# Bhumbra/probayes

Measured on AMD Instinct MI355X. Metric: MH chain-steps/sec (whole node), 10-dim model, 65 536 chains, 1/2/4/8 GPU, higher is better.
Workload: dtype f64; 1 GPU; cfg2: 10-dim diagonal-Gaussian random-walk MH, 65536 chains/GPU, full trace every step; chains_per_gpu=65536, dim=10, trace=True, steps_per_launch=250, parallelism=chain-sharded x1

## Files before the change

### include/pbhip.h

```cpp
#ifndef PBHIP_H
#define PBHIP_H

#include <stdint.h>

#ifdef __cplusplus
extern "C" {
#endif

#define PBH_ABI_VERSION 7
#define PBH_ABI_REVISION 2
#define PBH_MAX_DIM 32

#define PBH_OK 0
#define PBH_ERR_ARG (-1)
#define PBH_ERR_HIP (-2)
#define PBH_ERR_STATE (-3)
#define PBH_ERR_UNSUPPORTED (-4)
#define PBH_ERR_RCCL (-5)

enum pbh_target_kind {
  PBH_TARGET_DIAG_GAUSS = 1,
  PBH_TARGET_NORM_IID = 2,
  PBH_TARGET_GMM = 3,
  PBH_TARGET_NORM_PDF = 4,
// ... 138 lines not shown
int pbh_upload_replay(pbh_engine *eng, int64_t n_steps, const double *rand);
int pbh_stream_width(pbh_engine *eng, int32_t *r);
int pbh_legacy_seed(pbh_engine *eng, const uint32_t *seeds);
int pbh_legacy_replay(pbh_engine *eng, int64_t n_steps);
int pbh_reserve_replay(pbh_engine *eng, int64_t n_steps);
int pbh_get_replay(pbh_engine *eng, int64_t first, int64_t n_steps,
                   int32_t draw, double *out);
int pbh_legacy_run(pbh_engine *eng, int64_t n_steps, int32_t steps_per_launch);
int pbh_set_record_threshold(pbh_engine *eng, int32_t on);
int pbh_get_thresholds(pbh_engine *eng, int64_t first, int64_t n_steps, double *out);
enum pbh_draws { PBH_DRAWS_GAUSS = 0, PBH_DRAWS_LINREG = 1 };
int pbh_legacy_draws(pbh_engine *eng, int64_t n_steps, int64_t step0, int32_t kind,
                     double param, double *out);

enum { PBH_TRACE_NOFILL = 0x100 };
int pbh_alloc_trace(pbh_engine *eng, int64_t capacity, int32_t thin,
                    int32_t debug);
int pbh_run(pbh_engine *eng, int64_t n_steps, int32_t steps_per_launch);
int pbh_sync(pbh_engine *eng);
int pbh_run_wait(pbh_engine *eng, int64_t n_steps, int32_t steps_per_launch);
int pbh_set_collect(pbh_engine *eng, int32_t flags);
int pbh_last_run_ms(pbh_engine *eng, double *ms, int64_t *launches);
int pbh_server_stop(pbh_engine *eng);
int pbh_server_info(pbh_engine *eng, int32_t *active, int64_t *commands,
                    int64_t *launches);
int pbh_server_stamps(pbh_engine *eng, int32_t cap, uint32_t *seq, uint64_t *t0,
                      uint64_t *t1, int32_t *n);

int pbh_get_state(pbh_engine *eng, double *x, double *logp);
int pbh_trace_len(pbh_engine *eng, int64_t *n_recorded);
int pbh_get_trace(pbh_engine *eng, int64_t first, int64_t n, double *x,
                  double *logp, uint64_t *acc, double *p_x, double *p_p,
                  double *s);
int pbh_get_moments(pbh_engine *eng, double *sum, double *sumsq,
                    int64_t *n_acc, int64_t *n_steps);
int pbh_reset_moments(pbh_engine *eng);
int pbh_trace_ess(pbh_engine *eng, int64_t first, int64_t count, double *ess);
int pbh_trace_ess_total(pbh_engine *eng, int64_t first, int64_t count, double *total);
int pbh_trace_stats(pbh_engine *eng, int64_t first, int64_t count, double *sum,
                    double *sumsq, int64_t *n_acc);
int pbh_trace_expectation(pbh_engine *eng, int64_t first, int64_t count,
                          double exponent, double *out);
#define PBH_QUANTILE_MAX_RECORDS 2048
#define PBH_QUANTILE_MAX_Q 64
int pbh_trace_quantile(pbh_engine *eng, int64_t first, int64_t count,
                       int32_t nq, const double *q, int32_t weighted,
                       double *out);
int pbh_trace_rhat(pbh_engine *eng, int64_t first, int64_t count, int32_t group,
                   double *split_rhat, double *nested_rhat, double *chain_stats);
int pbh_trace_quantile_pooled(pbh_engine *eng, int64_t first, int64_t count,
                              int32_t nq, const double *q, double *out,
                              double *order_stats);

int pbh_trace_rhat_rank(pbh_engine *eng, int64_t first, int64_t count,
                        double *bulk, double *folded, double *ranks,
                        double *folded_ranks);

#define PBH_ESS_RANK_MAX_HALF 2048
int pbh_trace_ess_rank(pbh_engine *eng, int64_t first, int64_t count,
                       double *bulk, double *tail, double *tail_parts,
                       double *basic, double *mean_acov);

int pbh_rccl_unique_id(uint8_t id[128]);
int pbh_rccl_init(pbh_engine *eng, int32_t rank, int32_t world,
                  const uint8_t id[128]);
int pbh_rccl_max_chains(pbh_engine *eng, int64_t *n_max);
// ... 41 lines not shown
```

### probayes_amd/_lib.py

```python
import ctypes
import os

_HERE = os.path.dirname(os.path.abspath(__file__))
LIB_PATH = os.environ.get('PBHIP_LIB', os.path.join(_HERE, 'libpbhip.so'))

ABI_VERSION = 7
ABI_REVISION = 2
DRAWS_GAUSS, DRAWS_LINREG = 0, 1
MAX_DIM = 32

TARGET = {'diag_gauss': 1, 'norm_iid': 2, 'gmm': 3, 'norm_pdf': 4,
          'uniform_pdf': 5, 'mvn': 6, 'expr': 7}
PSCALE = {'log': 0, 'lin': 1}
SCORES = {'hastings': 1, 'metropolis': 2, 'gibbs': 3}
TRAN = {'const': 1, 'gauss_pdf': 2}
PROPOSAL = {'gauss': 1, 'sphere': 2, 'uniform': 3, 'gibbs': 4, 'vardelta': 5}
VAR_FIXED, VAR_POLARITY, VAR_UNIFORM, VAR_RANDINT = 0, 1, 2, 3
RNG = {'replay': 0, 'philox': 1, 'philox_f64': 2, 'xoshiro': 3,
       'philox_fp32': 4}
COLLECT_MOMENTS = 1

_dp = ctypes.POINTER(ctypes.c_double)
_ip = ctypes.POINTER(ctypes.c_int32)
_u8p = ctypes.POINTER(ctypes.c_uint8)
# ... 61 lines not shown
    'pbh_upload_replay': (ctypes.c_int, [ctypes.c_void_p, ctypes.c_int64, _dp]),
    'pbh_stream_width': (ctypes.c_int, [ctypes.c_void_p, _ip]),
    'pbh_legacy_seed': (ctypes.c_int, [ctypes.c_void_p, _u32p]),
    'pbh_legacy_replay': (ctypes.c_int, [ctypes.c_void_p, ctypes.c_int64]),
    'pbh_reserve_replay': (ctypes.c_int, [ctypes.c_void_p, ctypes.c_int64]),
    'pbh_legacy_run': (ctypes.c_int, [ctypes.c_void_p, ctypes.c_int64, ctypes.c_int32]),
    'pbh_set_record_threshold': (ctypes.c_int, [ctypes.c_void_p, ctypes.c_int32]),
    'pbh_get_thresholds': (ctypes.c_int, [ctypes.c_void_p, ctypes.c_int64,
                                          ctypes.c_int64, _dp]),
    'pbh_legacy_draws': (ctypes.c_int, [ctypes.c_void_p, ctypes.c_int64, ctypes.c_int64,
                                        ctypes.c_int32, ctypes.c_double, _dp]),
    'pbh_get_replay': (ctypes.c_int, [ctypes.c_void_p, ctypes.c_int64,
                                      ctypes.c_int64, ctypes.c_int32, _dp]),
    'pbh_alloc_trace': (ctypes.c_int, [ctypes.c_void_p, ctypes.c_int64,
                                       ctypes.c_int32, ctypes.c_int32]),
    'pbh_run': (ctypes.c_int, [ctypes.c_void_p, ctypes.c_int64, ctypes.c_int32]),
    'pbh_sync': (ctypes.c_int, [ctypes.c_void_p]),
    'pbh_run_wait': (ctypes.c_int, [ctypes.c_void_p, ctypes.c_int64, ctypes.c_int32]),
    'pbh_trace_ess_total': (ctypes.c_int, [ctypes.c_void_p, ctypes.c_int64,
                                           ctypes.c_int64, _dp]),
    'pbh_set_collect': (ctypes.c_int, [ctypes.c_void_p, ctypes.c_int32]),
    'pbh_last_run_ms': (ctypes.c_int, [ctypes.c_void_p, _dp, _i64p]),
    'pbh_server_stop': (ctypes.c_int, [ctypes.c_void_p]),
    'pbh_get_chain_logs': (ctypes.c_int, [ctypes.c_void_p, _dp, _ip]),
    'pbh_set_chain_logs': (ctypes.c_int, [ctypes.c_void_p, _dp]),
    'pbh_server_info': (ctypes.c_int, [ctypes.c_void_p, _ip, _i64p, _i64p]),
    'pbh_server_stamps': (ctypes.c_int, [ctypes.c_void_p, ctypes.c_int32, _u32p,
                                         _u64p, _u64p, _ip]),
    'pbh_get_state': (ctypes.c_int, [ctypes.c_void_p, _dp, _dp]),
    'pbh_trace_len': (ctypes.c_int, [ctypes.c_void_p, _i64p]),
    'pbh_get_trace': (ctypes.c_int, [ctypes.c_void_p, ctypes.c_int64,
                                     ctypes.c_int64, _dp, _dp, _u64p, _dp, _dp,
                                     _dp]),
    'pbh_get_moments': (ctypes.c_int, [ctypes.c_void_p, _dp, _dp, _i64p, _i64p]),
    'pbh_reset_moments': (ctypes.c_int, [ctypes.c_void_p]),
    'pbh_trace_stats': (ctypes.c_int, [ctypes.c_void_p, ctypes.c_int64,
                                       ctypes.c_int64, _dp, _dp, _i64p]),
    'pbh_rccl_unique_id': (ctypes.c_int, [_u8p]),
    'pbh_rccl_init': (ctypes.c_int, [ctypes.c_void_p, ctypes.c_int32,
                                     ctypes.c_int32, _u8p]),
    'pbh_rccl_max_chains': (ctypes.c_int, [ctypes.c_void_p, _i64p]),
    'pbh_rccl_allgather_stats': (ctypes.c_int, [ctypes.c_void_p, _dp, _i64p]),
    'pbh_get_checkpoint': (ctypes.c_int, [ctypes.c_void_p, _dp, _dp,
                                          ctypes.POINTER(ctypes.c_int64),
                                          ctypes.POINTER(ctypes.c_int32),
                                          _u32p]),
    'pbh_restore': (ctypes.c_int, [ctypes.c_void_p, _dp, _dp, ctypes.c_int64,
                                   ctypes.c_int32, _u32p]),
    'pbh_set_chains': (ctypes.c_int, [ctypes.c_void_p, _dp, _dp, ctypes.c_int64,
                                      ctypes.c_int32]),
    'pbh_legacy_state_words': (ctypes.c_int, [ctypes.c_void_p,
                                              ctypes.POINTER(ctypes.c_int64)]),
    'pbh_get_legacy_state': (ctypes.c_int, [ctypes.c_void_p, _u32p, _i32p, _i32p,
                                            _dp]),
    'pbh_set_legacy_state': (ctypes.c_int, [ctypes.c_void_p, _u32p, _i32p, _i32p,
                                            _dp]),
    'pbh_trace_expectation': (ctypes.c_int, [ctypes.c_void_p, ctypes.c_int64,
                                             ctypes.c_int64, ctypes.c_double,
                                             _dp]),
    'pbh_trace_quantile': (ctypes.c_int, [ctypes.c_void_p, ctypes.c_int64,
                                          ctypes.c_int64, ctypes.c_int32, _dp,
                                          ctypes.c_int32, _dp]),
    'pbh_trace_rhat': (ctypes.c_int, [ctypes.c_void_p, ctypes.c_int64,
                                      ctypes.c_int64, ctypes.c_int32, _dp, _dp,
                                      _dp]),
    'pbh_trace_quantile_pooled': (ctypes.c_int, [ctypes.c_void_p, ctypes.c_int64,
# ... 82 lines not shown
```

### probayes_amd/csrc/pbh_device.h

```cpp
#pragma once
#include <hip/hip_runtime.h>
#include <stdint.h>

#include "pbh_philox.h"

namespace pbh {

constexpr double kNearlyPosZero = 2.2250738585072014e-308;
constexpr double kNearlyPosInf = 1.7976931348623158e+308;
constexpr double kNearlyNegInf = -1.7976931348623158e+308;


__device__ __forceinline__ u32x4 philox4x32_10(u32x4 c, uint32_t k0,
                                                uint32_t k1) {
  constexpr uint32_t M0 = 0xD2511F53u, M1 = 0xCD9E8D57u;
  constexpr uint32_t W0 = 0x9E3779B9u, W1 = 0xBB67AE85u;
#pragma unroll
  for (int i = 0; i < 10; ++i) {
    const uint64_t p0 = (uint64_t)M0 * c.x;
    const uint64_t p1 = (uint64_t)M1 * c.z;
    const uint32_t hi0 = (uint32_t)(p0 >> 32), lo0 = (uint32_t)p0;
    const uint32_t hi1 = (uint32_t)(p1 >> 32), lo1 = (uint32_t)p1;
    c = u32x4{(uint32_t)__builtin_amdgcn_bitop3_b32(hi1, c.y, k0, 0x96), lo1,
              (uint32_t)__builtin_amdgcn_bitop3_b32(hi0, c.w, k1, 0x96), lo0};
// ... 365 lines not shown
}

__device__ __forceinline__ void st_buf(double *base, uint32_t voff,
                                       uint32_t soff, double v) {
  typedef unsigned int u32x2_t __attribute__((__vector_size__(8)));
  const __amdgpu_buffer_rsrc_t rs =
      __builtin_amdgcn_make_buffer_rsrc(base, 0, -1, 0x00020000);
  __builtin_amdgcn_raw_buffer_store_b64(__builtin_bit_cast(u32x2_t, v), rs,
                                        (int)voff, (int)soff, 2);
}

constexpr uint32_t kNoStore = 0x80000000u;
__device__ __forceinline__ void st_buf_n(double *base, uint32_t nbytes,
                                         uint32_t voff, double v) {
  typedef unsigned int u32x2_t __attribute__((__vector_size__(8)));
  const __amdgpu_buffer_rsrc_t rs =
      __builtin_amdgcn_make_buffer_rsrc(base, 0, (int)nbytes, 0x00020000);
  __builtin_amdgcn_raw_buffer_store_b64(__builtin_bit_cast(u32x2_t, v), rs,
                                        (int)voff, 0, 2);
}
__device__ __forceinline__ void st_buf_ns(double *base, uint32_t nbytes, uint32_t voff,
                                          uint32_t soff, double v) {
  typedef unsigned int u32x2_t __attribute__((__vector_size__(8)));
  const __amdgpu_buffer_rsrc_t rs =
      __builtin_amdgcn_make_buffer_rsrc(base, 0, (int)nbytes, 0x00020000);
  __builtin_amdgcn_raw_buffer_store_b64(__builtin_bit_cast(u32x2_t, v), rs,
                                        (int)voff, (int)soff, 2);
}
__device__ __forceinline__ void st_buf32_n(uint32_t *base, uint32_t nbytes,
                                           uint32_t voff, uint32_t v) {
  const __amdgpu_buffer_rsrc_t rs =
      __builtin_amdgcn_make_buffer_rsrc(base, 0, (int)nbytes, 0x00020000);
  __builtin_amdgcn_raw_buffer_store_b32(v, rs, (int)voff, 0, 0);
}

__device__ __forceinline__ uint32_t sel_u32(uint64_t m, uint32_t if0, uint32_t if1) {
  uint32_t r;
  asm("v_cndmask_b32_e64 %0, %1, %2, %3" : "=v"(r) : "v"(if0), "v"(if1), "s"(m));
  return r;
}
__device__ __forceinline__ double sel_f64(uint64_t m, double if0, double if1) {
  const uint64_t a = __builtin_bit_cast(uint64_t, if0), b = __builtin_bit_cast(uint64_t, if1);
  const uint32_t lo = sel_u32(m, (uint32_t)a, (uint32_t)b);
  const uint32_t hi = sel_u32(m, (uint32_t)(a >> 32), (uint32_t)(b >> 32));
  return __builtin_bit_cast(double, ((uint64_t)hi << 32) | lo);
}
__device__ __forceinline__ float sel_f32(uint64_t m, float if0, float if1) {
  return __builtin_bit_cast(float, sel_u32(m, __builtin_bit_cast(uint32_t, if0),
                                           __builtin_bit_cast(uint32_t, if1)));
}

__device__ __forceinline__ double lo_closed(double lo, bool incl) {
  if (incl || lo != lo) return lo;
  if (lo == __builtin_inf()) return __builtin_nan("");
  if (lo == 0.) return 0x1p-1074;
  const int64_t b = __builtin_bit_cast(int64_t, lo);
  return __builtin_bit_cast(double, lo > 0. ? b + 1 : b - 1);
}
__device__ __forceinline__ double hi_closed(double hi, bool incl) {
  if (incl || hi != hi) return hi;
  if (hi == -__builtin_inf()) return __builtin_nan("");
  if (hi == 0.) return -0x1p-1074;
  const int64_t b = __builtin_bit_cast(int64_t, hi);
  return __builtin_bit_cast(double, hi > 0. ? b - 1 : b + 1);
}

// ... 313 lines not shown
```

### probayes_amd/csrc/pbh_kernels_impl.h

```cpp
#pragma once
#include <utility>

#include "pbh_kernels.h"
#include "pbh_device.h"
#include "../../include/pbhip.h"

namespace pbh {

namespace {

constexpr int kBlock = 256;
constexpr int kPairFullBlock = 512;

__device__ __forceinline__ double cld(const double *p, int64_t i) {
  return ((const __attribute__((address_space(4))) double *)p)[i];
}

__device__ __forceinline__ double uni(double v) {
  const uint64_t u = __builtin_bit_cast(uint64_t, v);
  const uint32_t lo = __builtin_amdgcn_readfirstlane((uint32_t)u);
  const uint32_t hi = __builtin_amdgcn_readfirstlane((uint32_t)(u >> 32));
  return __builtin_bit_cast(double, (uint64_t)lo | ((uint64_t)hi << 32));
}

// ... 1152 lines not shown
    double cA[H], cB[H];
    uint32_t ctA = 0, ctB = 0, t1 = 0;
    int s = 0;
    if constexpr (PD::F32) {
      double nA[H], nB[H];
      uint32_t ntA = 0, ntB = 0;
      PD::draw(a, s_bmt, h, a.g0 >> 1, chain, cA, cB, ctA, ctB);
      if ((a.g0 & 1) && s < a.n_steps) {
        step(s, cB, ctB, t1);
        ++s;
        if (s < a.n_steps)
          PD::draw(a, s_bmt, h, (a.g0 + s) >> 1, chain, cA, cB, ctA, ctB);
      }
      for (; s + 3 < a.n_steps; s += 4) {
        PD::draw(a, s_bmt, h, ((a.g0 + s) >> 1) + 1, chain, nA, nB, ntA, ntB);
        step(s, cA, ctA, t1);
        step(s + 1, cB, ctB, t1);
        PD::draw(a, s_bmt, h, ((a.g0 + s) >> 1) + 2, chain, cA, cB, ctA, ctB);
        step(s + 2, nA, ntA, t1);
        step(s + 3, nB, ntB, t1);
      }
      if (s + 1 < a.n_steps) {
        step(s, cA, ctA, t1);
        step(s + 1, cB, ctB, t1);
        s += 2;
        if (s < a.n_steps)
          PD::draw(a, s_bmt, h, (a.g0 + s) >> 1, chain, cA, cB, ctA, ctB);
      }
      if (s < a.n_steps) step(s, cA, ctA, t1);
    } else if constexpr (FULL) {
        int64_t g0v = a.g0;
        int32_t nsv = a.n_steps, fairv = a.fair, fair_relv = a.fair_rel;
        constexpr int NW = 3 * H + 1, NB = (NW + 3) / 4, QA = (H + 1) / 2;
        constexpr uint64_t kHi = 0xFFFFFFFF00000000ull;
        uint64_t inl = __ballot(__builtin_fabs(lp) <= 700.);
        const uint32_t lpoff = hi ? loff : kNoStore;
        const uint32_t lpbytes = (uint32_t)(a.n * 8);
        const uint32_t aoff = lane == 32 ? (uint32_t)((c >> 5) * 4) : kNoStore;
        const uint32_t abytes = (uint32_t)(a.W * 8);
        int64_t rec = g0v + s - a.rec_base;
        const PhiloxKeys rk = philox_keys_v(a.seed_lo, a.seed_hi);
        uint32_t pre_hi = (uint32_t)((uint64_t)g0v >> 33);
        PhiloxPrefix<NB> pre =
            philox_prefix<NB>(16u * (uint32_t)h, chain, pre_hi, a.seed_lo, a.seed_hi);
        auto philox_from = [&](int64_t P, uint32_t (&w)[4 * NB], auto Q0) {
          philox_prefix_blocks<NB, decltype(Q0)::value>((uint32_t)P, pre, rk, w);
        };
        auto philox = [&](int64_t P, uint32_t (&w)[4 * NB]) {
          philox_prefix_blocks<NB>((uint32_t)P, pre, rk, w);
        };
        auto normals = [&](const uint32_t (&w)[4 * NB], auto Q0, auto Q1,
                           double (&ra)[H], double (&rb)[H]) {
          constexpr int q0 = decltype(Q0)::value, q1 = decltype(Q1)::value;
#pragma unroll
          for (int q = q0; q < q1; ++q) {
            double z0, z1;
            bm96_pair(w[3 * q], w[3 * q + 1], w[3 * q + 2], s_bmt, z0, z1);
#pragma unroll
            for (int e = 0; e < 2; ++e) {
              const int n = 2 * q + e;
              const double z = e ? z1 : z0;
              if (n < H) ra[n] = z;
              else rb[n - H] = z;
            }
          }
        };
        auto step_full = [&](int si, const double (&r)[H], uint32_t t0) {
          double xp[H];
#pragma unroll
          for (int i = 0; i < H; ++i)
            xp[i] = LOC0 ? __builtin_fma(r[i], psc[i], x[i])
                         : x[i] + __builtin_fma(r[i], psc[i], plc[i]);
          double p0 = 0., p1 = 0.;
#pragma unroll
          for (int i = 0; i < H; ++i) {
            const double u = __builtin_fma(xp[i], cb[i], -ca[i]);
            if (i & 1) p1 = __builtin_fma(u, u, p1);
            else p0 = __builtin_fma(u, u, p0);
          }
          double lo, up;
          halves_f64(p0 + p1, lo, up);
          const double lpp = (-(lo + up)) - a.ksum;
          const float eL = __builtin_amdgcn_exp2f(
              (float)__builtin_fma(lpp - lp, 1.4426950408889634, 16.0));
          const float fl = (float)t0;
          const uint64_t inp = __ballot(__builtin_fabs(lpp) <= 700.);
          const uint64_t inr = inp & inl;
          const uint64_t af = __ballot(fl <= __builtin_fmaf(eL, 0.999996f, -1.0f));
          const uint64_t rf = __ballot(fl > eL * 1.000004f);
          uint64_t accm = inr & af;
          const uint64_t needm = ~(inr & (af | rf)) & kHi;
          if (needm) {
            bool ex = false;
            if (__builtin_amdgcn_inverse_ballot_w64(needm))
              ex = pair_exact(a.seed_lo, a.seed_hi, a.log_npi, g0v + si, chain, h,
                              t0, lpp, lp);
            accm = (accm & ~needm) | (__ballot(ex) & needm);
          }
          const uint64_t mhi = accm & kHi;
          const uint64_t macc = mhi | (mhi >> 32);
#pragma unroll
          for (int i = 0; i < H; ++i) x[i] = sel_f64(macc, x[i], xp[i]);
          lp = sel_f64(macc, lp, lpp);
          inl = (inl & ~macc) | (inp & macc);
          double *row = a.tx + rec * D * a.n;
#pragma unroll
          for (int i = 0; i < H; ++i) st_buf(row, boff, i * bstride, x[i]);
          st_buf_n(a.tlp + rec * a.n, lpbytes, lpoff, lp);
          st_buf32_n(reinterpret_cast<uint32_t *>(a.tacc + rec * a.W), abytes, aoff,
                     (uint32_t)(mhi >> 32));
          ++rec;
        };
        using I0 = std::integral_constant<int, 0>;
        using IA = std::integral_constant<int, QA>;
        using IH = std::integral_constant<int, H>;
        auto run_block = [&]() {
          if (g0v & 1) {
            constexpr int QB = 3 * (H / 2) / 4;
            uint32_t w[4 * NB];
            philox_from(g0v >> 1, w, std::integral_constant<int, QB>{});
            normals(w, std::integral_constant<int, H / 2>{}, IH{}, cA, cB);
            __builtin_amdgcn_s_waitcnt(0);
            step_full(0, cB, w[3 * H] & 0xFFFFu);
            s = 1;
          }
          if (s + 1 < nsv) {
            uint32_t w[4 * NB];
            philox((g0v + s) >> 1, w);
            normals(w, I0{}, IH{}, cA, cB);
            ctA = w[3 * H] >> 16;
            ctB = w[3 * H] & 0xFFFFu;
            if (s == 0) __builtin_amdgcn_s_waitcnt(0);
            PBH_PHASE(2);
            const uint32_t slot = fairv ? simd_wave_slot() : 0u;
            const uint64_t tfair0 =
                fair_relv ? __builtin_amdgcn_s_memrealtime() : 0ull;
            for (; s + 3 < nsv; s += 2) {
              if (fairv) {
                const int64_t el = (int64_t)(__builtin_amdgcn_s_memrealtime() - tfair0);
                fair_prio((uint32_t)((el > 0 ? (uint64_t)el : 0ull) >> fairv) + slot);
              }
              PBH_PHASE_Q(s >> 1, nsv >> 1);
              uint32_t nw[4 * NB];
              double nA[H], nB[H];
              philox(((g0v + s) >> 1) + 1, nw);
              step_full(s, cA, ctA);
              normals(nw, I0{}, IA{}, nA, nB);
              step_full(s + 1, cB, ctB);
              normals(nw, IA{}, IH{}, nA, nB);
  #pragma unroll
              for (int i = 0; i < H; ++i) {
                cA[i] = nA[i];
                cB[i] = nB[i];
              }
              ctA = nw[3 * H] >> 16;
              ctB = nw[3 * H] & 0xFFFFu;
            }
            step_full(s, cA, ctA);
            step_full(s + 1, cB, ctB);
            s += 2;
          }
          if (s < nsv) {
            uint32_t w[4 * NB];
            philox((g0v + s) >> 1, w);
            normals(w, I0{}, IA{}, cA, cB);
            if (s == 0) __builtin_amdgcn_s_waitcnt(0);
            step_full(s, cA, w[3 * H] >> 16);
          }
        };
        if constexpr (SRV) {
          __shared__ int64_t s_cmd[6];
          SrvCmd *const hcmd = reinterpret_cast<SrvCmd *>(a.srv_cmd);
          SrvCmd *const mail = reinterpret_cast<SrvCmd *>(a.srv_mail);
          SrvDone *const donep = reinterpret_cast<SrvDone *>(a.srv_done) + blockIdx.x;
          const bool poller = __builtin_amdgcn_readfirstlane((int)(threadIdx.x >> 6)) == 0;
          const bool direct = (a.srv_mode & 1) != 0;
          const bool relay = blockIdx.x == 0 && !direct;
          uint32_t seen = 0u;
          for (;;) {
            if (poller) {
              const uint64_t tw = __builtin_amdgcn_s_memrealtime();
              const SrvCmd *src = relay ? hcmd : mail;
              uint32_t q;
              u32x4v v;
              for (;;) {
                v = ld16_sys(src);
                q = (uint32_t)__builtin_amdgcn_readfirstlane((int)v.x);
                const uint32_t chk = (uint32_t)__builtin_amdgcn_readfirstlane((int)v.w) >> 24;
                if (q != seen && chk == (q & 0xFFu)) break;
                if (__builtin_amdgcn_s_memrealtime() - tw > (uint64_t)a.srv_idle) {
                  q = 0u;
                  break;
                }
                __builtin_amdgcn_s_sleep(1);
              }
              const uint64_t tsee = __builtin_amdgcn_s_memrealtime();
              if (relay && q) st16_sys(mail, v);
              const uint32_t n = (uint32_t)__builtin_amdgcn_readfirstlane((int)v.y);
              const uint64_t arg =
                  (uint64_t)(uint32_t)__builtin_amdgcn_readfirstlane((int)v.z) |
                  ((uint64_t)(uint32_t)__builtin_amdgcn_readfirstlane((int)v.w) << 32);
              const int64_t g0 = (int64_t)(arg & 0xFFFFFFFFFFFFull);
              const uint32_t fr = (uint32_t)(arg >> 48) & 31u, frel = (uint32_t)(arg >> 53) & 1u;
              const uint32_t op = (uint32_t)(arg >> 54) & 1u;
              s_cmd[0] = q;
              s_cmd[1] = op;
              s_cmd[2] = g0;
              s_cmd[3] = n;
              s_cmd[4] = ((int64_t)frel << 32) | fr;
              s_cmd[5] = (int64_t)tsee;
            }
            __syncthreads();
            const uint32_t q = (uint32_t)__builtin_amdgcn_readfirstlane((int)s_cmd[0]);
            const uint32_t op = (uint32_t)__builtin_amdgcn_readfirstlane((int)s_cmd[1]);
            if (q == 0u || op == kSrvExit) {
              if (poller && q != 0u)
                __hip_atomic_store(&donep->seq, q, __ATOMIC_RELAXED, __HIP_MEMORY_SCOPE_SYSTEM);
              break;
            }
            const int64_t c2 = s_cmd[2], c4 = s_cmd[4];
            g0v = (int64_t)(uint32_t)__builtin_amdgcn_readfirstlane((int)(uint32_t)c2) |
                  ((int64_t)__builtin_amdgcn_readfirstlane((int)(c2 >> 32)) << 32);
            nsv = __builtin_amdgcn_readfirstlane((int)s_cmd[3]);
            fairv = __builtin_amdgcn_readfirstlane((int)(uint32_t)c4);
            fair_relv = __builtin_amdgcn_readfirstlane((int)(c4 >> 32));
            const uint64_t tseen = (uint64_t)s_cmd[5];
            s = 0;
            rec = g0v - a.rec_base;
            if ((uint32_t)((uint64_t)g0v >> 33) != pre_hi) {
              pre_hi = (uint32_t)((uint64_t)g0v >> 33);
              pre = philox_prefix<NB>(16u * (uint32_t)h, chain, pre_hi, a.seed_lo, a.seed_hi);
            }
            run_block();
            __builtin_amdgcn_s_waitcnt(0);
            __syncthreads();
            if (poller) {
              __hip_atomic_store(&donep->t0, tseen, __ATOMIC_RELAXED, __HIP_MEMORY_SCOPE_SYSTEM);
              __hip_atomic_store(&donep->t1, (uint64_t)__builtin_amdgcn_s_memrealtime(),
                                 __ATOMIC_RELAXED, __HIP_MEMORY_SCOPE_SYSTEM);
              __builtin_amdgcn_s_waitcnt(0);
              __hip_atomic_store(&donep->seq, q, __ATOMIC_RELAXED, __HIP_MEMORY_SCOPE_SYSTEM);
            }
            seen = q;
          }
        } else {
          run_block();
        }
        PBH_PHASE(3);
    } else {
      if (a.g0 & 1) {
        PD::draw(a, s_bmt, h, a.g0 >> 1, chain, cA, cB, ctA, ctB);
        step(s, cB, ctB, t1);
        ++s;
      }
      for (; s + 1 < a.n_steps; s += 2) {
        PD::draw(a, s_bmt, h, (a.g0 + s) >> 1, chain, cA, cB, ctA, ctB);
        step(s, cA, ctA, t1);
        step(s + 1, cB, ctB, t1);
      }
      if (s < a.n_steps) {
        PD::draw(a, s_bmt, h, (a.g0 + s) >> 1, chain, cA, cB, ctA, ctB);
// ... 1201 lines not shown
      a.gq[(p * M + ii) * a.n + c] = st.go[ii];
    }
    if (p == 0) {
      a.lp[c] = st.lp;
      if (a.moments) a.nacc[c] += a.n_steps;
      a.gq[D * a.n + c] = st.Q;
    }
  }
}

}

template <int D, int TGT, int PROP>
void launch_mh_spec(const KArgs &a, hipStream_t st, size_t lds) {
  const dim3 grid((unsigned)((a.n + kBlock - 1) / kBlock)), block(kBlock);
  if (a.rng == PBH_RNG_REPLAY)
    pbh_launch((mh_kernel<D, PBH_RNG_REPLAY, TGT, PROP>), grid, block,
                       lds, st, a);
  else if (a.rng == PBH_RNG_PHILOX)
    pbh_launch((mh_kernel<D, PBH_RNG_PHILOX, TGT, PROP>), grid, block,
                       lds, st, a);
  else if (a.rng == PBH_RNG_XOSHIRO)
    pbh_launch((mh_kernel<D, PBH_RNG_XOSHIRO, TGT, PROP>), grid, block,
                       lds, st, a);
  else
    pbh_launch((mh_kernel<D, PBH_RNG_PHILOX_F64, TGT, PROP>), grid,
                       block, lds, st, a);
}

inline bool pair_full_form(const KArgs &a) {
  return a.pair_full && a.rng == PBH_RNG_PHILOX && a.has_pred && a.thin == 1 &&
         a.pscale != PBH_PSCALE_LIN && a.tx != nullptr && a.n % 32 == 0 &&
         a.n * 8 <= (int64_t)kNoStore &&
         a.g0 - a.rec_base >= 0 && a.g0 + a.n_steps - a.rec_base <= a.rec_cap &&
         pair_index_hi_const(a.g0, a.n_steps);
}

inline bool iid_full_form(const KArgs &a) {
  return a.iid_full && a.rng == PBH_RNG_PHILOX && a.simple_acc && !a.debug &&
         a.has_pred && a.thin == 1 && a.pscale != PBH_PSCALE_LIN && a.tx != nullptr &&
         !a.has_tfun && a.vint == 0 && a.bnd_on == 0 && !a.moments &&
         a.ufun < (1u << a.d) && a.n * 8 <= (int64_t)kNoStore &&
         (int64_t)a.n_steps * a.d * a.n * 8 <= (int64_t)kNoStore &&
         a.g0 - a.rec_base >= 0 && a.g0 + a.n_steps - a.rec_base <= a.rec_cap;
}

template <int D, bool MOM>
void launch_mh_pair_m(const KArgs &a, hipStream_t st, dim3 grid, dim3 block) {
  if constexpr (!MOM) {
    if (pair_full_form(a)) {
      if (a.ploc_zero)
        pbh_launch((mh_pair_kernel<D, PBH_RNG_PHILOX, false, true, true>), grid, block, 0, st, a);
      else
        pbh_launch((mh_pair_kernel<D, PBH_RNG_PHILOX, false, false, true>), grid, block, 0, st, a);
      return;
    }
  }
  if (a.rng == PBH_RNG_REPLAY)
    pbh_launch((mh_pair_kernel<D, PBH_RNG_REPLAY, MOM>), grid, block, 0, st, a);
  else if (a.rng == PBH_RNG_PHILOX && a.ploc_zero)
    pbh_launch((mh_pair_kernel<D, PBH_RNG_PHILOX, MOM, true>), grid, block, 0, st, a);
  else if (a.rng == PBH_RNG_PHILOX)
    pbh_launch((mh_pair_kernel<D, PBH_RNG_PHILOX, MOM>), grid, block, 0, st, a);
  else if (a.rng == PBH_RNG_XOSHIRO)
    pbh_launch((mh_pair_kernel<D, PBH_RNG_XOSHIRO, MOM>), grid, block, 0, st, a);
  else if (a.rng == PBH_RNG_PHILOX_FP32)
// ... 236 lines not shown
```

### probayes_amd/csrc/pbh_trace.cpp

```cpp
#include <algorithm>
#include <cmath>
#include <cstring>
#include <initializer_list>

#include "pbh_engine_state.h"
#include "pbh_trace_host.h"

using pbh::check_ptr;
using pbh::fail;

namespace {

struct NamedPtr {
  const void *p;
  const char *name;
};

constexpr char kRange[] = "trace range [%lld, %lld) outside [0, %lld)";
constexpr char kRangeEss[] = "ESS needs >= 2 records inside [0, %3$lld), got [%1$lld, %2$lld)";

template <class Own = int (*)()>
int trace_enter(pbh_engine *e, std::initializer_list<NamedPtr> ptrs, bool need_trace,
                int64_t first, int64_t count, int64_t min_count,
                Own own = [] { return PBH_OK; }, const char *range = kRange) {
// ... 77 lines not shown
  if (err == hipSuccess && rows)
    err = pbh::launch_rhat_chain(at<const double>(e->scratch, l.z), e->n, 1, 0, count,
                                 at<double>(e->scratch, l.stats), e->stream);
  return err;
}

}

extern "C" {

int pbh_trace_len(pbh_engine *e, int64_t *n_recorded) {
  if (check_ptr(e, "engine") || check_ptr(n_recorded, "n_recorded")) return PBH_ERR_ARG;
  const int64_t r = e->cap > 0 ? e->g / e->thin - e->rec_base : 0;
  *n_recorded = std::max<int64_t>(0, std::min(r, e->cap));
  return PBH_OK;
}

int pbh_get_trace(pbh_engine *e, int64_t first, int64_t cnt, double *x,
                  double *logp, uint64_t *acc, double *p_x, double *p_p,
                  double *s) {
  if (const int rc = trace_enter(e, {}, false, first, cnt, 0)) return rc;
  if ((p_x || p_p || s) && !e->debug)
    return fail(PBH_ERR_STATE, "debug trace not allocated");
  HIP_TRY(hipSetDevice(e->device));
  HIP_TRY(hipStreamSynchronize(e->stream));
  const size_t n = e->n, d = e->d, W = (e->n + 63) / 64;
  if (cnt == 0) return PBH_OK;
  if (x) HIP_TRY(hipMemcpy(x, e->tx + first * d * n, cnt * d * n * sizeof(double), hipMemcpyDeviceToHost));
  if (logp) HIP_TRY(hipMemcpy(logp, e->tlp + first * n, cnt * n * sizeof(double), hipMemcpyDeviceToHost));
  if (acc) HIP_TRY(hipMemcpy(acc, e->tacc + first * W, cnt * W * sizeof(uint64_t), hipMemcpyDeviceToHost));
  if (p_x) HIP_TRY(hipMemcpy(p_x, e->tpx + first * d * n, cnt * d * n * sizeof(double), hipMemcpyDeviceToHost));
  if (p_p) HIP_TRY(hipMemcpy(p_p, e->tpp + first * n, cnt * n * sizeof(double), hipMemcpyDeviceToHost));
  if (s) HIP_TRY(hipMemcpy(s, e->ts + first * n, cnt * n * sizeof(double), hipMemcpyDeviceToHost));
  return PBH_OK;
}

int pbh_trace_stats(pbh_engine *e, int64_t first, int64_t count, double *sum,
                    double *sumsq, int64_t *n_acc) {
  if (const int rc = trace_enter(e, {}, false, first, count, 0)) return rc;
  HIP_TRY(hipSetDevice(e->device));
  const int64_t n = e->n, W = (n + 63) / 64;
  HIP_TRY(pbh::launch_trace_stats(e->tx, e->tacc, n, e->d, W, first, count,
                                  e->msum, e->msq, e->nacc, e->stream));
  HIP_TRY(hipStreamSynchronize(e->stream));
  e->mom_steps = count;
  const size_t dn = (size_t)e->d * n;
  if (sum) HIP_TRY(hipMemcpy(sum, e->msum, dn * sizeof(double), hipMemcpyDeviceToHost));
  if (sumsq) HIP_TRY(hipMemcpy(sumsq, e->msq, dn * sizeof(double), hipMemcpyDeviceToHost));
  if (n_acc) HIP_TRY(hipMemcpy(n_acc, e->nacc, n * sizeof(int64_t), hipMemcpyDeviceToHost));
  return PBH_OK;
}

int pbh_trace_expectation(pbh_engine *e, int64_t first, int64_t count,
                          double exponent, double *out) {
  if (const int rc = trace_enter(e, {{out, "out"}}, false, first, count, 1)) return rc;
  if (!std::isfinite(exponent)) return fail(PBH_ERR_ARG, "exponent must be finite");
  HIP_TRY(hipSetDevice(e->device));
  const size_t dn = (size_t)e->d * e->n;
  if (const int rc = scratch(e, dn * sizeof(double))) return rc;
  double *dout = at<double>(e->scratch, 0);
  hipError_t err = pbh::launch_trace_expectation(
      e->tx, e->tlp, e->n, e->d, first, count, exponent,
      e->k.pscale == PBH_PSCALE_LIN ? 1 : 0, e->k.log_npi, dout, e->stream);
  if (err == hipSuccess) err = hipStreamSynchronize(e->stream);
  if (err == hipSuccess)
    err = hipMemcpy(out, dout, dn * sizeof(double), hipMemcpyDeviceToHost);
// ... 293 lines not shown
```

### probayes_amd/engine.py

```python
import atexit
import ctypes
import weakref

import numpy as np
import scipy.stats

from probayes_amd import _lib
from probayes_amd.spec import normalize_spec

_c = ctypes


def _dp(a):
  return a.ctypes.data_as(_c.POINTER(_c.c_double))


def _ip(a):
  return a.ctypes.data_as(_c.POINTER(_c.c_int32))


def _f64(a):
  return np.ascontiguousarray(a, dtype=np.float64)


# ... 231 lines not shown
      raise ValueError('replay stream shape {} does not match R={}, N={}'
                       .format(streams.shape, self.stream_width(), self.n))
    _lib.call('pbh_upload_replay', self._h, _c.c_int64(T), _dp(streams))

  def seed_legacy(self, seeds):
    seeds = np.ascontiguousarray(np.asarray(seeds).reshape(-1), dtype=np.int64)
    if seeds.size != self.n:
      raise ValueError('need {} seeds, got {}'.format(self.n, seeds.size))
    if np.any(seeds < 0) or np.any(seeds > 0xFFFFFFFF):
      raise ValueError('Seed must be between 0 and 2**32 - 1')
    s32 = np.ascontiguousarray(seeds.astype(np.uint32))
    _lib.call('pbh_legacy_seed', self._h,
              s32.ctypes.data_as(_c.POINTER(_c.c_uint32)))

  def legacy_replay(self, n_steps):
    _lib.call('pbh_legacy_replay', self._h, _c.c_int64(int(n_steps)))

  def reserve_replay(self, n_steps):
    _lib.call('pbh_reserve_replay', self._h, _c.c_int64(int(n_steps)))

  def get_replay(self, first, n_steps, draw=-1):
    r = self.stream_width()
    shape = (n_steps, r, self.n) if draw < 0 else (n_steps, self.n)
    out = np.empty(shape, np.float64)
    _lib.call('pbh_get_replay', self._h, _c.c_int64(int(first)),
              _c.c_int64(int(n_steps)), int(draw), _dp(out))
    return out

  def alloc_trace(self, capacity, thin=1, debug=False, fill=True):
    flags = (1 if debug else 0) | (0 if fill else 0x100)
    _lib.call('pbh_alloc_trace', self._h, _c.c_int64(int(capacity)),
              int(thin), flags)
    self.debug = bool(debug)

  def run(self, n_steps, steps_per_launch=0, sync=True):
    fn = self._fn_run_wait if sync else self._fn_run
    rc = fn(self._h, int(n_steps), int(steps_per_launch))
    if rc:
      _lib.raise_status('pbh_run_wait' if sync else 'pbh_run', rc)

  def legacy_run(self, n_steps, steps_per_launch=0, sync=True):
    _lib.call('pbh_legacy_run', self._h, _c.c_int64(int(n_steps)),
              int(steps_per_launch))
    if sync:
      self.sync()

  def set_record_threshold(self, on=True):
    _lib.call('pbh_set_record_threshold', self._h, 1 if on else 0)

  def get_thresholds(self, first, n_steps):
    out = np.empty((int(n_steps), self.n), np.float64)
    _lib.call('pbh_get_thresholds', self._h, _c.c_int64(int(first)),
              _c.c_int64(int(n_steps)), _dp(out))
    return out

  def legacy_draws(self, n_steps, step0=0, kind='linreg', param=1.0):
    k = {'gauss': _lib.DRAWS_GAUSS, 'linreg': _lib.DRAWS_LINREG}[kind]
    out = np.empty((int(n_steps), self.n), np.float64)
    _lib.call('pbh_legacy_draws', self._h, _c.c_int64(int(n_steps)),
              _c.c_int64(int(step0)), k, _c.c_double(float(param)), _dp(out))
    return out

  def sync(self):
    rc = self._fn_sync(self._h)
    if rc:
      _lib.raise_status('pbh_sync', rc)
# ... 122 lines not shown
      _lib.call('pbh_set_legacy_state', self._h, key.ctypes.data_as(_lib._u32p),
                pos.ctypes.data_as(_lib._i32p), has.ctypes.data_as(_lib._i32p),
                _dp(gauss))

  def trace_len(self):
    r = _c.c_int64()
    _lib.call('pbh_trace_len', self._h, _c.byref(r))
    return r.value

  def _window(self, first, count):
    return first, self.trace_len() - first if count is None else count

  def trace(self, first=0, count=None, debug=None):
    first, count = self._window(first, count)
    n, d = self.n, self.dim
    W = (n + 63) // 64
    x = np.empty((count, d, n))
    lp = np.empty((count, n))
    acc = np.empty((count, W), np.uint64)
    debug = self.debug if debug is None else debug
    px = np.empty((count, d, n)) if debug else None
    pp = np.empty((count, n)) if debug else None
    sc = np.empty((count, n)) if debug else None
    nul = _c.POINTER(_c.c_double)()
    _lib.call('pbh_get_trace', self._h, _c.c_int64(first), _c.c_int64(count),
              _dp(x), _dp(lp), acc.ctypes.data_as(_c.POINTER(_c.c_uint64)),
              _dp(px) if debug else nul, _dp(pp) if debug else nul,
              _dp(sc) if debug else nul)
    out = {'v_x': x.transpose(2, 0, 1), 'v_p': lp.T, 'u': unpack_accept(acc, n)}
    if debug:
      out.update({'p_x': px.transpose(2, 0, 1), 'p_p': pp.T, 's': sc.T})
    return out

  def moments(self):
    n, d = self.n, self.dim
    s = np.empty((d, n))
    q = np.empty((d, n))
    na = np.empty(n, np.int64)
    steps = _c.c_int64()
    _lib.call('pbh_get_moments', self._h, _dp(s), _dp(q),
              na.ctypes.data_as(_c.POINTER(_c.c_int64)), _c.byref(steps))
    return {'sum': s.T.copy(), 'sumsq': q.T.copy(), 'n_acc': na,
            'n_steps': steps.value}

  def trace_stats(self, first=0, count=None):
    first, count = self._window(first, count)
    n, d = self.n, self.dim
    s = np.empty((d, n))
    q = np.empty((d, n))
    na = np.empty(n, np.int64)
    _lib.call('pbh_trace_stats', self._h, _c.c_int64(int(first)),
              _c.c_int64(int(count)), _dp(s), _dp(q),
              na.ctypes.data_as(_c.POINTER(_c.c_int64)))
    return {'sum': s.T.copy(), 'sumsq': q.T.copy(), 'n_acc': na,
            'n_steps': int(count)}

  def reset_moments(self):
    _lib.call('pbh_reset_moments', self._h)

  @staticmethod
  def rccl_unique_id():
    buf = (_c.c_uint8 * 128)()
    _lib.call('pbh_rccl_unique_id', buf)
    return bytes(buf)

  def rccl_init(self, rank, world, uid):
# ... 138 lines not shown
```

Before: 48.43 billion chain-steps/s.

## Use persistent buffer resources with scalar offsets for trace stores; unroll step pairs

Trace stores now use buffer resource descriptors built once and advanced through scalar (SGPR) offsets each step, with precomputed per-dim lane offsets. This replaces rebuilding 64-bit row pointers every step, and the descriptor is rebased only when the scalar offset would overflow. Ballot masks are narrowed to 32-bit upper halves kept in scalar registers via readfirstlane, and the main loop is unrolled to two Philox pairs per iteration for small H. This aims to cut address arithmetic and VGPR pressure in the store-heavy trace path. It also adds a host API to copy the whole trace buffer and a launch guard that keeps offsets within 32 bits.

New measurement: 48.21 billion chain-steps/s. About the same (-0.5%).

```diff
diff --git a/include/pbhip.h b/include/pbhip.h
--- a/include/pbhip.h
+++ b/include/pbhip.h
@@ -194,6 +194,7 @@
 int pbh_get_trace(pbh_engine *eng, int64_t first, int64_t n, double *x,
                   double *logp, uint64_t *acc, double *p_x, double *p_p,
                   double *s);
+int pbh_get_trace_buffer(pbh_engine *eng, double *x, double *logp, uint64_t *acc);
 int pbh_get_moments(pbh_engine *eng, double *sum, double *sumsq,
                     int64_t *n_acc, int64_t *n_steps);
 int pbh_reset_moments(pbh_engine *eng);
diff --git a/probayes_amd/_lib.py b/probayes_amd/_lib.py
--- a/probayes_amd/_lib.py
+++ b/probayes_amd/_lib.py
@@ -117,6 +117,7 @@
     'pbh_get_trace': (ctypes.c_int, [ctypes.c_void_p, ctypes.c_int64,
                                      ctypes.c_int64, _dp, _dp, _u64p, _dp, _dp,
                                      _dp]),
+    'pbh_get_trace_buffer': (ctypes.c_int, [ctypes.c_void_p, _dp, _dp, _u64p]),
     'pbh_get_moments': (ctypes.c_int, [ctypes.c_void_p, _dp, _dp, _i64p, _i64p]),
     'pbh_reset_moments': (ctypes.c_int, [ctypes.c_void_p]),
     'pbh_trace_stats': (ctypes.c_int, [ctypes.c_void_p, ctypes.c_int64,
diff --git a/probayes_amd/csrc/pbh_device.h b/probayes_amd/csrc/pbh_device.h
--- a/probayes_amd/csrc/pbh_device.h
+++ b/probayes_amd/csrc/pbh_device.h
@@ -421,6 +421,26 @@
   const __amdgpu_buffer_rsrc_t rs =
       __builtin_amdgcn_make_buffer_rsrc(base, 0, (int)nbytes, 0x00020000);
   __builtin_amdgcn_raw_buffer_store_b32(v, rs, (int)voff, 0, 0);
+}
+
+__device__ __forceinline__ uint32_t opaque_s(uint32_t v) {
+  v = (uint32_t)__builtin_amdgcn_readfirstlane((int)v);
+  asm("" : "+s"(v));
+  return v;
+}
+
+__device__ __forceinline__ __amdgpu_buffer_rsrc_t trace_rsrc(void *base, uint32_t nbytes) {
+  return __builtin_amdgcn_make_buffer_rsrc(base, 0, (int)nbytes, 0x00020000);
+}
+__device__ __forceinline__ void st_rsrc(__amdgpu_buffer_rsrc_t rs, uint32_t voff,
+                                        uint32_t soff, double v) {
+  typedef unsigned int u32x2_t __attribute__((__vector_size__(8)));
+  __builtin_amdgcn_raw_buffer_store_b64(__builtin_bit_cast(u32x2_t, v), rs,
+                                        (int)voff, (int)soff, 2);
+}
+__device__ __forceinline__ void st_rsrc32(__amdgpu_buffer_rsrc_t rs, uint32_t voff,
+                                          uint32_t soff, uint32_t v) {
+  __builtin_amdgcn_raw_buffer_store_b32(v, rs, (int)voff, (int)soff, 0);
 }
 
 __device__ __forceinline__ uint32_t sel_u32(uint64_t m, uint32_t if0, uint32_t if1) {
diff --git a/probayes_amd/csrc/pbh_kernels_impl.h b/probayes_amd/csrc/pbh_kernels_impl.h
--- a/probayes_amd/csrc/pbh_kernels_impl.h
+++ b/probayes_amd/csrc/pbh_kernels_impl.h
@@ -1208,22 +1208,35 @@
         int64_t g0v = a.g0;
         int32_t nsv = a.n_steps, fairv = a.fair, fair_relv = a.fair_rel;
         constexpr int NW = 3 * H + 1, NB = (NW + 3) / 4, QA = (H + 1) / 2;
-        constexpr uint64_t kHi = 0xFFFFFFFF00000000ull;
-        uint64_t inl = __ballot(__builtin_fabs(lp) <= 700.);
+        uint32_t inl = (uint32_t)(__ballot(__builtin_fabs(lp) <= 700.) >> 32);
         const uint32_t lpoff = hi ? loff : kNoStore;
-        const uint32_t lpbytes = (uint32_t)(a.n * 8);
-        const uint32_t aoff = lane == 32 ? (uint32_t)((c >> 5) * 4) : kNoStore;
-        const uint32_t abytes = (uint32_t)(a.W * 8);
-        int64_t rec = g0v + s - a.rec_base;
+        const uint32_t aoff = lane == 32 && active ? (uint32_t)((c >> 5) * 4) : kNoStore;
+        constexpr bool kLaneDims = H <= 8;
+        uint32_t xoffk[kLaneDims ? H : 1];
+#pragma unroll
+        for (int i = 0; i < (kLaneDims ? H : 1); ++i) xoffk[i] = boff + (uint32_t)i * bstride;
+        const uint32_t rowx = (uint32_t)D * bstride, rowl = bstride;
+        const uint32_t rowa = (uint32_t)(a.W * 8);
+        const uint32_t xlim = 0xFFFFFF00u - rowx;
+        __amdgpu_buffer_rsrc_t rsx, rsl, rsa;
+        uint32_t sox, sol, soa;
+        auto rebase = [&](int sb, int k) {
+          const int64_t rec = g0v + ((int)opaque_s((uint32_t)sb) + k) - a.rec_base;
+          rsx = trace_rsrc(a.tx + rec * D * a.n, 0xFFFFFFFFu);
+          rsl = trace_rsrc(a.tlp + rec * a.n, kNoStore);
+          rsa = trace_rsrc(a.tacc + rec * a.W, kNoStore);
+          sox = sol = soa = 0u;
+        };
+        rebase(0, 0);
         const PhiloxKeys rk = philox_keys_v(a.seed_lo, a.seed_hi);
         uint32_t pre_hi = (uint32_t)((uint64_t)g0v >> 33);
         PhiloxPrefix<NB> pre =
             philox_prefix<NB>(16u * (uint32_t)h, chain, pre_hi, a.seed_lo, a.seed_hi);
-        auto philox_from = [&](int64_t P, uint32_t (&w)[4 * NB], auto Q0) {
-          philox_prefix_blocks<NB, decltype(Q0)::value>((uint32_t)P, pre, rk, w);
+        auto philox_from = [&](uint32_t P, uint32_t (&w)[4 * NB], auto Q0) {
+          philox_prefix_blocks<NB, decltype(Q0)::value>(P, pre, rk, w);
         };
-        auto philox = [&](int64_t P, uint32_t (&w)[4 * NB]) {
-          philox_prefix_blocks<NB>((uint32_t)P, pre, rk, w);
+        auto philox = [&](uint32_t P, uint32_t (&w)[4 * NB]) {
+          philox_prefix_blocks<NB>(P, pre, rk, w);
         };
         auto normals = [&](const uint32_t (&w)[4 * NB], auto Q0, auto Q1,
                            double (&ra)[H], double (&rb)[H]) {
@@ -1241,7 +1254,10 @@
             }
           }
         };
-        auto step_full = [&](int si, const double (&r)[H], uint32_t t0) {
+        using I0 = std::integral_constant<int, 0>;
+        using IA = std::integral_constant<int, QA>;
+        using IH = std::integral_constant<int, H>;
+        auto step_full = [&](int sb, int k, const double (&r)[H], uint32_t t0) {
           double xp[H];
 #pragma unroll
           for (int i = 0; i < H; ++i)
@@ -1260,88 +1276,112 @@
           const float eL = __builtin_amdgcn_exp2f(
               (float)__builtin_fma(lpp - lp, 1.4426950408889634, 16.0));
           const float fl = (float)t0;
-          const uint64_t inp = __ballot(__builtin_fabs(lpp) <= 700.);
-          const uint64_t inr = inp & inl;
-          const uint64_t af = __ballot(fl <= __builtin_fmaf(eL, 0.999996f, -1.0f));
-          const uint64_t rf = __ballot(fl > eL * 1.000004f);
-          uint64_t accm = inr & af;
-          const uint64_t needm = ~(inr & (af | rf)) & kHi;
-          if (needm) {
+          const uint32_t inp = (uint32_t)(__ballot(__builtin_fabs(lpp) <= 700.) >> 32);
+          const uint32_t inr = inp & inl;
+          const uint32_t af =
+              (uint32_t)(__ballot(fl <= __builtin_fmaf(eL, 0.999996f, -1.0f)) >> 32);
+          const uint32_t rf = (uint32_t)(__ballot(fl > eL * 1.000004f) >> 32);
+          uint32_t acch = inr & af;
+          const uint32_t needh = opaque_s(~(inr & (af | rf)));
+          if (needh) {
             bool ex = false;
-            if (__builtin_amdgcn_inverse_ballot_w64(needm))
-              ex = pair_exact(a.seed_lo, a.seed_hi, a.log_npi, g0v + si, chain, h,
+            if (__builtin_amdgcn_inverse_ballot_w64((uint64_t)needh << 32))
+              ex = pair_exact(a.seed_lo, a.seed_hi, a.log_npi,
+                              g0v + ((int)opaque_s((uint32_t)sb) + k), chain, h,
                               t0, lpp, lp);
-            accm = (accm & ~needm) | (__ballot(ex) & needm);
+            acch = (acch & ~needh) | ((uint32_t)(__ballot(ex) >> 32) & needh);
           }
-          const uint64_t mhi = accm & kHi;
-          const uint64_t macc = mhi | (mhi >> 32);
+          acch = opaque_s(acch);
+          const uint64_t macc = ((uint64_t)acch << 32) | acch;
 #pragma unroll
           for (int i = 0; i < H; ++i) x[i] = sel_f64(macc, x[i], xp[i]);
           lp = sel_f64(macc, lp, lpp);
-          inl = (inl & ~macc) | (inp & macc);
-          double *row = a.tx + rec * D * a.n;
-#pragma unroll
-          for (int i = 0; i < H; ++i) st_buf(row, boff, i * bstride, x[i]);
-          st_buf_n(a.tlp + rec * a.n, lpbytes, lpoff, lp);
-          st_buf32_n(reinterpret_cast<uint32_t *>(a.tacc + rec * a.W), abytes, aoff,
-                     (uint32_t)(mhi >> 32));
-          ++rec;
+          inl = (inl & ~acch) | (inp & acch);
+          if (sox > xlim) rebase(sb, k);
+#pragma unroll
+          for (int i = 0; i < H; ++i)
+            st_rsrc(rsx, xoffk[kLaneDims ? i : 0],
+                    kLaneDims ? sox : sox + (uint32_t)i * bstride, x[i]);
+          st_rsrc(rsl, lpoff, sol, lp);
+          st_rsrc32(rsa, aoff, soa, acch);
+          sox += rowx;
+          sol += rowl;
+          soa += rowa;
         };
-        using I0 = std::integral_constant<int, 0>;
-        using IA = std::integral_constant<int, QA>;
-        using IH = std::integral_constant<int, H>;
+        auto pair_body = [&](int sb, int k, uint32_t P1, const double (&ca_)[H],
+                             const double (&cb_)[H], uint32_t cta, uint32_t ctb,
+                             double (&na_)[H], double (&nb_)[H], uint32_t &nta,
+                             uint32_t &ntb) {
+          uint32_t nw[4 * NB];
+          philox(P1, nw);
+          step_full(sb, k, ca_, cta);
+          normals(nw, I0{}, IA{}, na_, nb_);
+          step_full(sb, k + 1, cb_, ctb);
+          normals(nw, IA{}, IH{}, na_, nb_);
+          nta = nw[3 * H] >> 16;
+          ntb = nw[3 * H] & 0xFFFFu;
+        };
         auto run_block = [&]() {
+          uint32_t P = (uint32_t)((uint64_t)g0v >> 1);
           if (g0v & 1) {
             constexpr int QB = 3 * (H / 2) / 4;
             uint32_t w[4 * NB];
-            philox_from(g0v >> 1, w, std::integral_constant<int, QB>{});
+            philox_from(P, w, std::integral_constant<int, QB>{});
             normals(w, std::integral_constant<int, H / 2>{}, IH{}, cA, cB);
             __builtin_amdgcn_s_waitcnt(0);
-            step_full(0, cB, w[3 * H] & 0xFFFFu);
+            step_full(0, 0, cB, w[3 * H] & 0xFFFFu);
             s = 1;
+            ++P;
           }
           if (s + 1 < nsv) {
             uint32_t w[4 * NB];
-            philox((g0v + s) >> 1, w);
+            philox(P, w);
             normals(w, I0{}, IH{}, cA, cB);
             ctA = w[3 * H] >> 16;
             ctB = w[3 * H] & 0xFFFFu;
             if (s == 0) __builtin_amdgcn_s_waitcnt(0);
             PBH_PHASE(2);
             const uint32_t slot = fairv ? simd_wave_slot() : 0u;
-            const uint64_t tfair0 =
-                fair_relv ? __builtin_amdgcn_s_memrealtime() : 0ull;
-            for (; s + 3 < nsv; s += 2) {
-              if (fairv) {
-                const int64_t el = (int64_t)(__builtin_amdgcn_s_memrealtime() - tfair0);
-                fair_prio((uint32_t)((el > 0 ? (uint64_t)el : 0ull) >> fairv) + slot);
-              }
+            const uint32_t tfair0 =
+                fair_relv ? (uint32_t)__builtin_amdgcn_s_memrealtime() : 0u;
+            constexpr bool kTwoPairs = H <= 6;
+            double nA[H], nB[H];
+            uint32_t ntA = 0, ntB = 0;
+            for (; kTwoPairs && s + 5 < nsv; s += 4) {
+              const uint32_t tnow = (uint32_t)__builtin_amdgcn_s_memrealtime();
               PBH_PHASE_Q(s >> 1, nsv >> 1);
-              uint32_t nw[4 * NB];
-              double nA[H], nB[H];
-              philox(((g0v + s) >> 1) + 1, nw);
-              step_full(s, cA, ctA);
-              normals(nw, I0{}, IA{}, nA, nB);
-              step_full(s + 1, cB, ctB);
-              normals(nw, IA{}, IH{}, nA, nB);
-  #pragma unroll
+              pair_body(s, 0, P + 1, cA, cB, ctA, ctB, nA, nB, ntA, ntB);
+              if (fairv) fair_prio(((tnow - tfair0) >> fairv) + slot);
+              PBH_PHASE_Q((s >> 1) + 1, nsv >> 1);
+              pair_body(s, 2, P + 2, nA, nB, ntA, ntB, cA, cB, ctA, ctB);
+              P += 2;
+            }
+            while (s + 3 < nsv) {
+              if (!kTwoPairs && fairv)
+                fair_prio((((uint32_t)__builtin_amdgcn_s_memrealtime() - tfair0) >> fairv) + slot);
+              if (!kTwoPairs) PBH_PHASE_Q(s >> 1, nsv >> 1);
+              pair_body(s, 0, P + 1, cA, cB, ctA, ctB, nA, nB, ntA, ntB);
+#pragma unroll
               for (int i = 0; i < H; ++i) {
                 cA[i] = nA[i];
                 cB[i] = nB[i];
               }
-              ctA = nw[3 * H] >> 16;
-              ctB = nw[3 * H] & 0xFFFFu;
+              ctA = ntA;
+              ctB = ntB;
+              s += 2;
+              ++P;
             }
-            step_full(s, cA, ctA);
-            step_full(s + 1, cB, ctB);
+            step_full(s, 0, cA, ctA);
+            step_full(s, 1, cB, ctB);
             s += 2;
+            ++P;
           }
           if (s < nsv) {
             uint32_t w[4 * NB];
-            philox((g0v + s) >> 1, w);
+            philox(P, w);
             normals(w, I0{}, IA{}, cA, cB);
             if (s == 0) __builtin_amdgcn_s_waitcnt(0);
-            step_full(s, cA, w[3 * H] >> 16);
+            step_full(s, 0, cA, w[3 * H] >> 16);
           }
         };
         if constexpr (SRV) {
@@ -1402,7 +1442,7 @@
             fair_relv = __builtin_amdgcn_readfirstlane((int)(c4 >> 32));
             const uint64_t tseen = (uint64_t)s_cmd[5];
             s = 0;
-            rec = g0v - a.rec_base;
+            rebase(0, 0);
             if ((uint32_t)((uint64_t)g0v >> 33) != pre_hi) {
               pre_hi = (uint32_t)((uint64_t)g0v >> 33);
               pre = philox_prefix<NB>(16u * (uint32_t)h, chain, pre_hi, a.seed_lo, a.seed_hi);
@@ -2670,6 +2710,7 @@
   return a.pair_full && a.rng == PBH_RNG_PHILOX && a.has_pred && a.thin == 1 &&
          a.pscale != PBH_PSCALE_LIN && a.tx != nullptr && a.n % 32 == 0 &&
          a.n * 8 <= (int64_t)kNoStore &&
+         (int64_t)a.d * a.n * 8 <= 0xFFFFFF00ll &&
          a.g0 - a.rec_base >= 0 && a.g0 + a.n_steps - a.rec_base <= a.rec_cap &&
          pair_index_hi_const(a.g0, a.n_steps);
 }
diff --git a/probayes_amd/csrc/pbh_trace.cpp b/probayes_amd/csrc/pbh_trace.cpp
--- a/probayes_amd/csrc/pbh_trace.cpp
+++ b/probayes_amd/csrc/pbh_trace.cpp
@@ -133,6 +133,17 @@
   if (p_x) HIP_TRY(hipMemcpy(p_x, e->tpx + first * d * n, cnt * d * n * sizeof(double), hipMemcpyDeviceToHost));
   if (p_p) HIP_TRY(hipMemcpy(p_p, e->tpp + first * n, cnt * n * sizeof(double), hipMemcpyDeviceToHost));
   if (s) HIP_TRY(hipMemcpy(s, e->ts + first * n, cnt * n * sizeof(double), hipMemcpyDeviceToHost));
+  return PBH_OK;
+}
+
+int pbh_get_trace_buffer(pbh_engine *e, double *x, double *logp, uint64_t *acc) {
+  if (const int rc = trace_enter(e, {}, true, 0, 0, 0)) return rc;
+  HIP_TRY(hipSetDevice(e->device));
+  HIP_TRY(hipStreamSynchronize(e->stream));
+  const size_t n = e->n, d = e->d, W = (e->n + 63) / 64, cap = e->cap;
+  if (x) HIP_TRY(hipMemcpy(x, e->tx, cap * d * n * sizeof(double), hipMemcpyDeviceToHost));
+  if (logp) HIP_TRY(hipMemcpy(logp, e->tlp, cap * n * sizeof(double), hipMemcpyDeviceToHost));
+  if (acc) HIP_TRY(hipMemcpy(acc, e->tacc, cap * W * sizeof(uint64_t), hipMemcpyDeviceToHost));
   return PBH_OK;
 }
 
diff --git a/probayes_amd/engine.py b/probayes_amd/engine.py
--- a/probayes_amd/engine.py
+++ b/probayes_amd/engine.py
@@ -287,6 +287,7 @@
     _lib.call('pbh_alloc_trace', self._h, _c.c_int64(int(capacity)),
               int(thin), flags)
     self.debug = bool(debug)
+    self.trace_cap = int(capacity)
 
   def run(self, n_steps, steps_per_launch=0, sync=True):
     fn = self._fn_run_wait if sync else self._fn_run
@@ -475,6 +476,15 @@
       out.update({'p_x': px.transpose(2, 0, 1), 'p_p': pp.T, 's': sc.T})
     return out
 
+  def trace_buffer(self):
+    n, d, capacity = self.n, self.dim, self.trace_cap
+    x = np.empty((capacity, d, n))
+    lp = np.empty((capacity, n))
+    acc = np.empty((capacity, (n + 63) // 64), np.uint64)
+    _lib.call('pbh_get_trace_buffer', self._h, _dp(x), _dp(lp),
+              acc.ctypes.data_as(_c.POINTER(_c.c_uint64)))
+    return x, lp, acc
+
   def moments(self):
     n, d = self.n, self.dim
     s = np.empty((d, n))
```
